# rwth-i6/rasr

Hardware: AMD Instinct MI355X
Metric: acoustic frames scored/sec (1e4-state AM) (higher is better)
Workload: dtype f16+mxfp6 (per f32 product: one f16 MFMA product + one block-scaled fp6 x fp6 MFMA product for both cross terms, f32 accumulate)

## Files before the change

include/amx.h:

```cpp
#ifndef RASR_AMD_AMX_H
#define RASR_AMD_AMX_H

#include <stddef.h>
#include <stdint.h>

#ifdef __cplusplus
extern "C" {
#endif

typedef enum {
    AMX_OK              = 0,
    AMX_ERR_INVALID     = -1,
    AMX_ERR_UNSUPPORTED = -2,
    AMX_ERR_DEVICE      = -3,
    AMX_ERR_STATE       = -4
} amx_status;

typedef struct amx_ctx  amx_ctx;
typedef struct amx_mfcc amx_mfcc;
typedef struct amx_mfcc_plan amx_mfcc_plan;
typedef struct amx_gmm  amx_gmm;
typedef struct amx_ffnn amx_ffnn;


// ... 289 lines not shown
    int                 n_pre;
    const int*          pre_type;
    const float* const* pre_mean;
    const float* const* pre_stddev;
    const int*          maxout_groups;
    const int* const*   maxout_sizes;
} amx_ffnn_layers;
int amx_ffnn_create_ex(amx_ctx* ctx, const amx_ffnn_model* model, const amx_ffnn_layers* ext, amx_ffnn** out);
void amx_ffnn_destroy(amx_ffnn* h);
int  amx_ffnn_input_dim(const amx_ffnn* h);
int  amx_ffnn_output_dim(const amx_ffnn* h);
int amx_ffnn_score(amx_ffnn* h, const float* feats_host, int T, float* scores_host);
int amx_ffnn_score_dev(amx_ffnn* h, const float* feats_dev, int feats_stride, int T, float* scores_dev);
int amx_ffnn_wait_dev(amx_ffnn* h);
int amx_ffnn_precision(const amx_ffnn* h, double* mx_block_ratio);
enum { AMX_NN_TOP_LINEAR = 0, AMX_NN_TOP_SOFTMAX = 1 };
int amx_ffnn_forward_dev(amx_ffnn* h, const float* feats_dev, int feats_stride, int T, float* out_dev, int top);
int amx_ffnn_score_stats_dev(amx_ffnn* h, const float* feats_dev, int feats_stride, int T, float* scores_dev,
                             uint32_t* best_state_dev, unsigned long long* state_counts_dev, double* score_sum_dev);

int amx_ffnn_hidden_dim(const amx_ffnn* h);
int amx_ffnn_forward_hidden_dev(amx_ffnn* h, const float* feats_dev, int feats_stride, int T, float* act_dev);
int amx_ffnn_score_on_demand_dev(amx_ffnn* h, const float* act_dev, int n_pairs, const uint32_t* frame_dev, const uint32_t* emission_dev,
                                 float* scores_dev);
int amx_precomputed_score_dev(amx_ctx* ctx, const float* feats_dev, int feats_stride, int T, int n_classes, const int* class_to_output_dev,
                              const float* log_prior_dev, float prior_scale, float* scores_dev);

int amx_class_labels_init(int n_classes, const int* disregard, int n_disregard, int* mapping, int* n_targets);
int amx_nn_vector_read_f32(const char* path, int* n, float** data);
int amx_nn_vector_write_f32(const char* path, int n, const float* data);
// ... 62 lines not shown
```

rasr_amd/_lib.py:

```python
import ctypes as C
import os

_HERE = os.path.dirname(os.path.abspath(__file__))
LIB_PATH = os.environ.get("AMX_LIBRARY", os.path.join(_HERE, "librasr_amd.so"))

AMX_OK, AMX_ERR_INVALID, AMX_ERR_UNSUPPORTED, AMX_ERR_DEVICE, AMX_ERR_STATE = 0, -1, -2, -3, -4
AMX_GMM_MAX, AMX_GMM_SUM, AMX_GMM_BATCH_FLOAT, AMX_GMM_SIMD, AMX_GMM_BATCH_INT, AMX_GMM_PRESELECTION_FLOAT, AMX_GMM_PRESELECTION_INT = 0, 1, 2, 3, 4, 5, 6
AMX_GMM_VITERBI, AMX_GMM_BAUM_WELCH = 0, 1
AMX_ACT_NONE, AMX_ACT_RELU, AMX_ACT_SIGMOID, AMX_ACT_TANH, AMX_ACT_ELU = 0, 1, 2, 3, 4
AMX_NN_PRE_LOGARITHM, AMX_NN_PRE_MEAN_AND_VARIANCE = 1, 2
AMX_NN_MAX_PRE = 4
AMX_PREC_FP32, AMX_PREC_BF16, AMX_PREC_BF16X3, AMX_PREC_F16MX = 0, 1, 2, 3
AMX_NN_TOP_LINEAR, AMX_NN_TOP_SOFTMAX = 0, 1
AMX_ARCHIVE_READ, AMX_ARCHIVE_WRITE = 0, 1
AMX_NORM_MEAN, AMX_NORM_MEAN_AND_VARIANCE = 0, 1


class AmxError(RuntimeError):
    def __init__(self, status, message):
        super().__init__("amx status %d: %s" % (status, message))
        self.status = status


class MfccCfg(C.Structure):
# ... 158 lines not shown
    "amx_pms_read": (C.c_int, [C.c_char_p, C.POINTER(_P)]),
    "amx_pms_write": (C.c_int, [C.POINTER(GmmModel), C.c_char_p]),
    "amx_mixture_set_view": (C.c_int, [_P, C.POINTER(GmmModel)]),
    "amx_mixture_set_destroy": (None, [_P]),
    "amx_ffnn_create": (C.c_int, [_P, C.POINTER(FfnnModel), C.POINTER(_P)]),
    "amx_ffnn_create_ex": (C.c_int, [_P, C.POINTER(FfnnModel), C.POINTER(FfnnLayers), C.POINTER(_P)]),
    "amx_ffnn_destroy": (None, [_P]),
    "amx_ffnn_input_dim": (C.c_int, [_P]),
    "amx_ffnn_output_dim": (C.c_int, [_P]),
    "amx_ffnn_score": (C.c_int, [_P, _P, C.c_int, _P]),
    "amx_ffnn_score_dev": (C.c_int, [_P, _P, C.c_int, C.c_int, _P]),
    "amx_device_clocks_dev": (C.c_int, [_P, _P]),
    "amx_device_clocks_xcd_dev": (C.c_int, [_P, _P]),
    "amx_ffnn_wait_dev": (C.c_int, [_P]),
    "amx_ffnn_precision": (C.c_int, [_P, C.POINTER(C.c_double)]),
    "amx_ffnn_score_stats_dev": (C.c_int, [_P, _P, C.c_int, C.c_int, _P, _P, _P, _P]),
    "amx_ffnn_hidden_dim": (C.c_int, [_P]),
    "amx_dc_detection": (C.c_int, [_P, C.c_longlong, C.c_double, C.c_double, C.c_float, C.c_double, C.c_int, C.c_int, _P, _P, C.c_longlong, _P]),
    "amx_ffnn_forward_hidden_dev": (C.c_int, [_P, _P, C.c_int, C.c_int, _P]),
    "amx_ffnn_forward_dev": (C.c_int, [_P, _P, C.c_int, C.c_int, _P, C.c_int]),
    "amx_ffnn_score_on_demand_dev": (C.c_int, [_P, _P, C.c_int, _P, _P, _P]),
    "amx_precomputed_score_dev": (C.c_int, [_P, _P, C.c_int, C.c_int, C.c_int, _P, _P, C.c_float, _P]),
    "amx_class_labels_init": (C.c_int, [C.c_int, _P, C.c_int, _P, C.POINTER(C.c_int)]),
    "amx_nn_vector_read_f32": (C.c_int, [C.c_char_p, C.POINTER(C.c_int), C.POINTER(_P)]),
    "amx_nn_vector_write_f32": (C.c_int, [C.c_char_p, C.c_int, _P]),
    "amx_nn_vector_read_s32": (C.c_int, [C.c_char_p, C.POINTER(C.c_int), C.POINTER(_P)]),
    "amx_nn_vector_write_s32": (C.c_int, [C.c_char_p, C.c_int, _P]),
    "amx_nn_vector_read_u32": (C.c_int, [C.c_char_p, C.POINTER(C.c_int), C.POINTER(_P)]),
    "amx_nn_matrix_read": (C.c_int, [C.c_char_p, C.POINTER(C.c_int), C.POINTER(C.c_int), C.POINTER(_P)]),
    "amx_nn_matrix_write": (C.c_int, [C.c_char_p, C.c_int, C.c_int, _P]),
# ... 59 lines not shown
```

rasr_amd/csrc/ffnn.hip:

```cpp
#include "common.hpp"

#include <hip/hip_bf16.h>

#include <algorithm>
#include <map>
#include <tuple>
#include <type_traits>
#include <cmath>
#include <cstring>

namespace amx {

typedef __attribute__((ext_vector_type(8))) short bf16x8;
typedef __attribute__((ext_vector_type(16))) float f32x16;
typedef unsigned short                              bf16_t;

typedef float  f32x2 __attribute__((ext_vector_type(2)));
typedef float  f32x4 __attribute__((ext_vector_type(4)));
typedef __bf16 bf16x2 __attribute__((ext_vector_type(2)));

__device__ __forceinline__ unsigned pack_bf16(float lo, float hi) {
    f32x2 v = {lo, hi};
    return __builtin_bit_cast(unsigned, __builtin_convertvector(v, bf16x2));
}
// ... 1325 lines not shown
        const void *feats, *scores, *best, *counts, *sum;
        hipStream_t stream;
        int         stride, T, stats;
        bool operator<(const GraphKey& o) const {
            return std::tie(feats, scores, best, counts, sum, stream, stride, T, stats) <
                   std::tie(o.feats, o.scores, o.best, o.counts, o.sum, o.stream, o.stride, o.T, o.stats);
        }
    };
    std::map<GraphKey, hipGraphExec_t> graphs;
    float *d_host_f = nullptr, *d_host_s = nullptr;
    size_t host_f_cap = 0, host_s_cap = 0;
    int    use_graphs = 1;
    int    gemm_persistent = 1;
    int    gemm_cfg       = -1;
    int    chunk          = 32768;
    int    mx_stagger     = 0;
    int    mx_dbg         = 0;
    int    mx_ksplit      = 1;
    float*    d_ks_ws  = nullptr;
    size_t    ks_ws_cap = 0;
    unsigned* h_overflow = nullptr;
    unsigned* d_overflow = nullptr;
    amx::PreOps         pre{};
    std::vector<float*> d_pre;
    std::vector<int>    mo_groups;
    std::vector<int*>   d_mo_off, d_mo_size;
    int    mo_width = 0;
    float* d_mo     = nullptr;
    size_t elt() const { return precision == AMX_PREC_FP32 ? 4 : 2; }
    bool   mfma_bf16() const { return precision != AMX_PREC_FP32; }
// ... 185 lines not shown
        case 11:
            if constexpr (LAST)
                launch_bf16<CfgS3, ACT, LAST>(h, l, x, ldx, out, ldo, T, Tpad);
            else
                launch_bf16<CfgS3L, ACT, LAST>(h, l, x, ldx, out, ldo, T, Tpad);
            break;
        default: launch_bf16<CfgA, ACT, LAST>(h, l, x, ldx, out, ldo, T, Tpad); break;
    }
}

using MfgL = amx::mx::MxCfg<256, 256, 2, 4, 3>;
using MfgLP = amx::mx::MxCfg<256, 256, 2, 4, 3, 4>;
using MfgLH = amx::mx::MxCfg<256, 256, 2, 4, 3, 0, 4>;
using MfgLF = amx::mx::MxCfg<256, 256, 2, 4, 3, 4, 4>;
using MfgLQ = amx::mx::MxCfg<256, 256, 2, 4, 3, 0, 0, 1, 0, 1>;
using MfgLW = amx::mx::MxCfg<256, 256, 2, 2, 3, 0, 0, 1, 0, 2>;
using MfgA = amx::mx::MxCfg<128, 128, 2, 2, 3>;
using MfgS = amx::mx::MxCfg<128, 64, 2, 2, 8, 0, 0, 2>;
using MfgS4 = amx::mx::MxCfg<128, 64, 2, 2, 4>;
using MfgSL = amx::mx::MxCfg<128, 64, 2, 2, 8, 0, 0, 2, 4>;
using MfgS8 = amx::mx::MxCfg<128, 64, 4, 2, 8, 0, 0, 2>;
using Mfg64 = amx::mx::MxCfg<64, 64, 2, 2, 8, 0, 0, 4, 4>;
using MfgSP = amx::mx::MxCfg<128, 64, 2, 2, 8, 0, 0, 2, 4, 3>;

template<class C, int ACT, bool LAST>
void launch_mx(amx_ffnn* h, int l, const void* x, int xkts, void* out, int ldo, int T, int Tpad, int n_valid) {
    const int ntn = h->Npad[l] / C::BN, ntt = Tpad / C::BT;
    const int gt = h->group_t >= 0 ? h->group_t : (C::BN == 256 ? 16 : 8), gn = h->group_n >= 0 ? h->group_n : (C::BN == 256 ? 8 : 2);
    constexpr int lds_bytes = amx::gemm_scratch_bytes<C, LAST>() + C::BN * 4;
    static_assert(lds_bytes <= 160 * 1024, "LDS budget");
// ... 96 lines not shown
            cfg = 8;
        else if (t128 >= ncu)
            cfg = 0;
        else if (t64 > ncu && t64 <= 2 * ncu)
            cfg = 6;
        else if (!LAST && 2 * t64 <= ncu && h->mx_ksplit <= 1)
            cfg = 14;
        else
            cfg = 3;
    }
    switch (cfg) {
        case 2: launch_mx<MfgL, ACT, LAST>(h, l, x, xkts, out, ldo, T, Tpad, n_valid); break;
        case 4: launch_mx<MfgLP, ACT, LAST>(h, l, x, xkts, out, ldo, T, Tpad, n_valid); break;
        case 5: launch_mx<MfgLH, ACT, LAST>(h, l, x, xkts, out, ldo, T, Tpad, n_valid); break;
        case 7: launch_mx<MfgLF, ACT, LAST>(h, l, x, xkts, out, ldo, T, Tpad, n_valid); break;
        case 8: launch_mx<MfgLQ, ACT, LAST>(h, l, x, xkts, out, ldo, T, Tpad, n_valid); break;
        case 9: launch_mx<MfgLW, ACT, LAST>(h, l, x, xkts, out, ldo, T, Tpad, n_valid); break;
        case 3:
            if constexpr (LAST)
                launch_mx<MfgS, ACT, LAST>(h, l, x, xkts, out, ldo, T, Tpad, n_valid);
            else
                launch_mx<MfgSP, ACT, LAST>(h, l, x, xkts, out, ldo, T, Tpad, n_valid);
            break;
        case 6: launch_mx<MfgS4, ACT, LAST>(h, l, x, xkts, out, ldo, T, Tpad, n_valid); break;
        case 12: launch_mx<MfgS8, ACT, LAST>(h, l, x, xkts, out, ldo, T, Tpad, n_valid); break;
        case 14:
            if constexpr (LAST)
                launch_mx<MfgS, ACT, LAST>(h, l, x, xkts, out, ldo, T, Tpad, n_valid);
            else
                launch_mx<Mfg64, ACT, LAST>(h, l, x, xkts, out, ldo, T, Tpad, n_valid);
            break;
// ... 89 lines not shown
        const amx::MaxoutSrc<decltype(a)::value> src{h->d_mo, h->out[l], h->d_mo_off[l], h->d_mo_size[l]};
        if (export_f32) {
            const int blocks = (int)std::min<long long>(4096, ((long long)Trows * Kp + 255) / 256);
            hipLaunchKernelGGL(amx::pack_input_f32<decltype(src)>, dim3(blocks), dim3(256), 0, h->ctx->stream, src, T, G, (float*)dst, Kp, Trows);
        }
        else
            pack_operand(h, src, T, G, dst, Kp, Trows);
    });
    AMX_HIP(hipGetLastError());
    return AMX_OK;
}

}

extern "C" {

int amx_ffnn_create(amx_ctx* ctx, const amx_ffnn_model* m, amx_ffnn** out) {
    return amx_ffnn_create_ex(ctx, m, nullptr, out);
}

int amx_ffnn_create_ex(amx_ctx* ctx, const amx_ffnn_model* m, const amx_ffnn_layers* ext, amx_ffnn** out) {
    AMX_REQUIRE(ctx && m && out, AMX_ERR_INVALID, "amx_ffnn_create: NULL argument");
    *out = nullptr;
    AMX_REQUIRE(m->n_layers >= 1 && m->in_dim && m->out_dim && m->W && m->bias && m->activation, AMX_ERR_INVALID,
                "amx_ffnn_create: empty network");
    AMX_REQUIRE(m->precision == AMX_PREC_FP32 || m->precision == AMX_PREC_BF16 || m->precision == AMX_PREC_BF16X3 ||
                        m->precision == AMX_PREC_F16MX,
                AMX_ERR_INVALID, "amx_ffnn_create: unknown precision");
    const int        n_pre = ext ? ext->n_pre : 0;
    std::vector<int> mo_groups((size_t)m->n_layers, 0);
// ... 84 lines not shown
            if (o < 0)
                continue;
            memcpy(&Wmap[(size_t)e * K], m->W[L0] + (size_t)o * K, (size_t)K * 4);
            bmap[e] = m->bias[L0] ? m->bias[L0][o] : 0.f;
            pmap[e] = m->log_prior ? m->log_prior[o] : 0.f;
        }
        out_dim[L0] = m->n_classes;
        Wl[L0]      = Wmap.data();
        bl[L0]      = bmap.data();
        if (m->log_prior)
            prior = pmap.data();
    }

    amx::Tuning tune;
    {
        static const char* const keys[] = {"tile", "graph", "persistent", "group", "chunk", "stagger", "mx_dbg", "mx_fallback", "ksplit", nullptr};
        if (!tune.parse(m->tuning, keys, "amx_ffnn_create"))
            return AMX_ERR_INVALID;
    }
    int t_tile, t_graph, t_persistent, t_chunk, t_mx_dbg, t_stagger, t_group_t = -1, t_group_n = -1, t_ksplit = 1;
    std::string t_mx_fallback;
    {
        const char* who = "amx_ffnn_create";
        static const char* const fallbacks[] = {"auto", "off", nullptr};
        if (!tune.get_word("mx_fallback", "auto", fallbacks, &t_mx_fallback, who) || !tune.get_int("ksplit", 1, 1, 4, &t_ksplit, who))
            return AMX_ERR_INVALID;
        AMX_REQUIRE(t_ksplit == 1 || t_ksplit == 4, AMX_ERR_INVALID, "amx_ffnn_create: tuning ksplit=%d: expected 1 | 4", t_ksplit);
        AMX_REQUIRE(t_ksplit == 1 || m->precision == AMX_PREC_F16MX, AMX_ERR_UNSUPPORTED, "amx_ffnn_create: tuning ksplit exists for AMX_PREC_F16MX only");
        if (!tune.get_int("tile", -1, -1, 14, &t_tile, who) || !tune.get_int("graph", 0, 0, 1, &t_graph, who) ||
            !tune.get_int("persistent", 1, 0, 1, &t_persistent, who) || !tune.get_int("chunk", 32768, 256, 1 << 24, &t_chunk, who) ||
            !tune.get_int("mx_dbg", 0, 0, 1 << 16, &t_mx_dbg, who) || !tune.get_int("stagger", 0, 0, 100000, &t_stagger, who))
            return AMX_ERR_INVALID;
        if (tune.has("group")) {
            const std::string g = tune.kv["group"];
            char              tail = 0;
            AMX_REQUIRE(sscanf(g.c_str(), "%dx%d%c", &t_group_t, &t_group_n, &tail) == 2 && t_group_t >= 1 && t_group_n >= 1 && t_group_t <= 4096 &&
                                t_group_n <= 4096,
                        AMX_ERR_INVALID, "amx_ffnn_create: tuning group=%s: expected <frame tiles>x<output tiles>, e.g. 16x8", g.c_str());
        }
    }
    int    prec = m->precision;
    double mx_ratio = 0.0;
    if (prec == AMX_PREC_F16MX) {
        for (int l = 0; l < m->n_layers; ++l) {
            const int    K = m->in_dim[l], N = out_dim[l];
            const float* W = Wl[l];
// ... 25 lines not shown
    }
    amx_ffnn* h  = new amx_ffnn;
    h->ctx       = ctx;
    h->n_layers  = m->n_layers;
    h->precision = prec;
    h->requested_precision = m->precision;
    h->mx_block_ratio      = mx_ratio;
    h->class_mapped = class_mapped;
    h->gemm_cfg        = t_tile;
    h->use_graphs      = t_graph;
    h->gemm_persistent = t_persistent;
    h->chunk           = t_chunk;
    h->mx_dbg          = t_mx_dbg;
    h->mx_stagger      = t_stagger;
    h->mx_ksplit       = t_ksplit;
    h->group_t         = t_group_t;
    h->group_n         = t_group_n;
    hipSetDevice(ctx->device);
    const int kmult = prec == AMX_PREC_F16MX ? amx::mx::TK : (prec != AMX_PREC_FP32) ? amx::BK : amx::FK;
    if (prec == AMX_PREC_F16MX) {
        if (hipHostMalloc((void**)&h->h_overflow, 4, hipHostMallocMapped) != hipSuccess ||
            hipHostGetDevicePointer((void**)&h->d_overflow, h->h_overflow, 0) != hipSuccess) {
            (void)hipGetLastError();
            amx::set_error("amx_ffnn_create: cannot allocate the overflow flag");
            amx_ffnn_destroy(h);
            return AMX_ERR_DEVICE;
        }
        *h->h_overflow = 0;
    }
    long      best_flops = -1;
// ... 565 lines not shown
```

rasr_amd/csrc/ffnn_mx.hpp:

```cpp
#pragma once

namespace amx {
namespace mx {

typedef _Float16 f16x8 __attribute__((ext_vector_type(8)));
typedef unsigned u32x4 __attribute__((ext_vector_type(4)));
typedef unsigned u32x2 __attribute__((ext_vector_type(2)));
typedef _Float16 f16x2 __attribute__((ext_vector_type(2)));
typedef _Float16 f16x16 __attribute__((ext_vector_type(16)));
typedef _Float16 f16x32 __attribute__((ext_vector_type(32)));
typedef float    f32v16 __attribute__((ext_vector_type(16)));
typedef unsigned u32x6 __attribute__((ext_vector_type(6)));
typedef int      v8i __attribute__((ext_vector_type(8)));

constexpr int TK    = 32;
constexpr int R_OFF = 16384;
constexpr int BLK   = 24576;

__host__ __device__ constexpr int pos16(int u) {
    return 8 * (2 * (u >> 4) + ((u >> 2) & 1)) + 4 * ((u >> 3) & 1) + (u & 3);
}
__host__ __device__ inline int h_off(int r, int c) {
    return r * 64 + ((c ^ ((r >> 2) & 3)) << 4);
}
__host__ __device__ inline int r_off(int r, int half) {
    return R_OFF + half * 4096 + r * 16;
}

__host__ __device__ inline int block_exponent(float max_abs) {
    unsigned u;
#if defined(__HIP_DEVICE_COMPILE__)
    u = __float_as_uint(max_abs);
#else
    memcpy(&u, &max_abs, 4);
#endif
    const int e = (int)((u >> 23) & 0xffu);
    return e < 14 ? 14 : e;
}

static inline unsigned fp6_code_host(float v, int sbyte) {
    const double a = std::fabs((double)v) * std::ldexp(1.0, 127 - sbyte);
// ... 2 lines not shown
        code = 31;
    else {
        const double step = a >= 4.0 ? 0.5 : a >= 2.0 ? 0.25 : 0.125;
        const double qv   = std::nearbyint(a / step) * step;
        if (qv >= 4.0)
            code = 24 + (unsigned)((qv - 4.0) / 0.5);
        else if (qv >= 2.0)
            code = 16 + (unsigned)((qv - 2.0) / 0.25);
        else
            code = (unsigned)(qv / 0.125);
    }
    return code | (std::signbit(v) ? 32u : 0u);
}

static inline void pack_weights_host(const float* W, int n_rows, int K, int ld, int Rpad, int KT, std::vector<unsigned char>& out) {
    out.assign((size_t)(Rpad / 256) * KT * BLK, 0);
    auto block_max = [&](int n, int kt) {
        float m = 0.f;
        if (n < n_rows)
            for (int u = 0; u < 32; ++u) {
                const int k = kt * 32 + u;
                if (k < K)
                    m = std::fmax(m, std::fabs(W[(size_t)n * ld + k]));
            }
        return m;
    };
    for (int n = 0; n < n_rows; ++n) {
        const int rb = n >> 8, r = n & 255;
        for (int kt = 0; kt < KT; ++kt) {
            unsigned char* blk = out.data() + ((size_t)rb * KT + kt) * BLK;
            float          v[32], lo[32];
            _Float16       hi[32];
            for (int u = 0; u < 32; ++u) {
                const int k = kt * 32 + u;
                v[u]        = k < K ? W[(size_t)n * ld + k] : 0.f;
                hi[u]       = (_Float16)v[u];
                lo[u]       = v[u] - (float)hi[u];
            }
            const int ec = block_exponent(std::fmax(block_max(n, kt), block_max(n ^ 32, kt)));
            unsigned  rec[2][4] = {{0, 0, 0, (unsigned)(ec - 2)}, {0, 0, 0, (unsigned)(ec - 2)}};
            for (int u = 0; u < 32; ++u) {
                const int p = pos16(u), chunk = p >> 3, half = chunk & 1, f = 8 * (chunk >> 1) + (p & 7);
                memcpy(blk + h_off(r, chunk) + (p & 7) * 2, &hi[u], 2);
                const unsigned code = fp6_code_host(lo[u], ec - 13);
                const int      bit = 6 * f, d = bit >> 5, sh = bit & 31;
                rec[half][d] |= code << sh;
                if (sh > 26)
                    rec[half][d + 1] |= code >> (32 - sh);
            }
            memcpy(blk + r_off(r, 0), rec[0], 16);
            memcpy(blk + r_off(r, 1), rec[1], 16);
        }
    }
}

struct LanePack {
    uint4 h0, h1, rec;
};

__device__ __forceinline__ unsigned pk_f16(float a, float b) {
    f16x2 v = {(_Float16)a, (_Float16)b};
    return __builtin_bit_cast(unsigned, v);
}

__device__ __forceinline__ LanePack lane_pack(const float (&a)[16], int ec, int sbyte) {
    LanePack o;
// ... 42 lines not shown
            }
        m = fmaxf(m, __shfl_xor(m, 1, 64));
        if (!(m < 65520.f))
            *overflow = 1u;
        const int ec = block_exponent(m);
        lane_store(out + ((size_t)(t >> 8) * KT + kt) * BLK, t & 255, hh, lane_pack(a, ec, ec - 13));
    }
}

template<int ACT>
__global__ __launch_bounds__(256) void neg_act_kernel(float* __restrict__ x, long long n) {
    for (long long i = (long long)blockIdx.x * 256 + threadIdx.x; i < n; i += (long long)gridDim.x * 256)
        x[i] = activate<ACT>(-x[i]);
}

template<int BN_, int BT_, int WN_, int WT_, int STAGES_, int PF_ = 0, int IW_ = 0, int U_ = 1, int LW_ = 0, int PIPE_ = 0>
struct MxCfg {
    static constexpr int BN = BN_, BT = BT_, WN = WN_, WT = WT_, STAGES = STAGES_;
    static constexpr int PIPE = PIPE_;
    static_assert(PIPE_ == 0 || (PIPE_ == 1 && U_ == 1 && LW_ == 0 && PF_ == 0 && IW_ == 0 && STAGES_ == 3 && WN_ * WT_ == 8) ||
                      (PIPE_ == 2 && U_ == 1 && LW_ == 0 && PF_ == 0 && IW_ == 0 && STAGES_ == 3 && WN_ * WT_ == 4 && BN_ / WN_ == 128 && BT_ / WT_ == 128) ||
                      (PIPE_ == 3 && U_ == 2 && LW_ > 0 && STAGES_ >= 2 * U_ + 1),
                  "ping-pong K loop: eight waves, every one of them issuing, plain three-stage ring; self-pipelined: four waves of 128 x 128; "
                  "read-ahead: loader waves, two K-tiles per barrier, a ring of at least three iterations");
    static constexpr int PF = PF_;
    static constexpr int U = U_;
    static_assert(U_ >= 1 && U_ <= 4 && STAGES_ >= 2 * U_, "ring: U K-tiles being read + at least U in flight");
    static_assert(PF_ == 0 || (BN_ == 256 && BT_ == 256 && WN_ * WT_ == 8), "the prefetch walks whole 256-row blocks with six waves");
    static constexpr int NW = WN * WT, LW = LW_, THREADS = (NW + LW_) * 64, PLANES = 1;
    static_assert(LW_ == 0 || (IW_ == 0 && PF_ == 0), "loader waves replace the issuing-wave variants");
    static constexpr bool SKEW = false, SPREAD = false;
    static constexpr int MI = BN / WN / 32, MJ = BT / WT / 32;
    static constexpr int A_R = BN * 64, A_BYTES = BN * 96;
    static constexpr int B_R = BT * 64, B_BYTES = BT * 96;
    static constexpr int STAGE_BYTES = A_BYTES + B_BYTES, LDS_BYTES = STAGES * STAGE_BYTES;
    static constexpr int A_PIECES = BN / 16 + BN / 32, B_PIECES = BT / 16 + BT / 32;
    static constexpr int TOTAL = A_PIECES + B_PIECES;
    static constexpr int IW  = LW_ > 0 ? LW_ : IW_ > 0 ? IW_ : NW;
    static constexpr int PPW = (TOTAL + IW - 1) / IW;
    static constexpr int NHI = TOTAL % IW;
    static constexpr bool PF_FREE = PF_ > 0 && IW_ > 0;
    static_assert(PF_ == 0 || IW_ == 0 || IW_ * 2 == WN_ * WT_, "free prefetch: half of the waves issue the DMA");
    static_assert(BN % 64 == 0 && BT % 64 == 0 && 256 % BN == 0 && 256 % BT == 0, "tiles are whole record pieces of a 256-row block");
    static_assert(STAGES >= 2 && STAGES <= 8 && (STAGES - 2) * (PPW + (PF_ > 0 ? 1 : 0)) + 1 < 64, "vmcnt immediate");
};

template<class C>
__device__ __forceinline__ void piece_offsets(int p, int ha, int hb, int& src, int& dst, bool& is_b) {
    is_b = p >= C::A_PIECES;
    if (!is_b) {
        if (p < C::BN / 16) {
            src = (ha * (C::BN / 16) + p) * 1024;
            dst = p * 1024;
        }
        else {
            const int j = p - C::BN / 16, half = j / (C::BN / 64), gq = j % (C::BN / 64);
            src = R_OFF + half * 4096 + (ha * (C::BN / 64) + gq) * 1024;
            dst = C::A_R + half * (C::BN * 16) + gq * 1024;
        }
    }
    else {
        const int q = p - C::A_PIECES;
        if (q < C::BT / 16) {
            src = (hb * (C::BT / 16) + q) * 1024;
            dst = C::A_BYTES + q * 1024;
// ... 105 lines not shown
            tile_n = 0;
        }
        auto tile_stamp = [&](int phase) {
#ifdef AMX_LAB
            if constexpr ((DBG & 2048) != 0) {
                const int nth = (vi - (int)blockIdx.x) / (int)gridDim.x;
                if (blockIdx.x == 0 && nth < 4 && tid == 0 && (!LAST || n_tiles_total > 1000)) {
                    mx_tile_stamps[(nth * 3 + phase) * 2]     = __builtin_amdgcn_s_memtime();
                    mx_tile_stamps[(nth * 3 + phase) * 2 + 1] = __builtin_amdgcn_s_memrealtime();
                }
            }
#endif
        };
        tile_stamp(0);
        const int   n0 = tile_n * C::BN, t0 = tile_t * C::BT;
        const char* wblk = W + (size_t)(n0 >> 8) * KT * BLK;
        const char* xblk = X + (size_t)(t0 >> 8) * xkts * BLK;
        const int   ha = (n0 & 255) / C::BN, hb = (t0 & 255) / C::BT;
        const int KT_all = KT;
        if (reduce)
            KT = 0;
        if (KSPLIT && ks > 1) {
            const int per = ((KT_all + ks - 1) / ks + C::U - 1) / C::U * C::U, kt_lo = min(kgroup * per, KT_all);
            KT   = min(per, KT_all - kt_lo);
            wblk += (size_t)kt_lo * BLK;
            xblk += (size_t)kt_lo * BLK;
        }

        int  p_src[C::PPW], p_dst[C::PPW];
        bool p_b[C::PPW];
#pragma unroll
        for (int q = 0; q < C::PPW; ++q) {
            const int p = q * C::IW + iwave;
            if (p < C::TOTAL && issuer)
                piece_offsets<C>(p, ha, hb, p_src[q], p_dst[q], p_b[q]);
            else {
                p_src[q] = p_dst[q] = 0;
                p_b[q]              = false;
            }
        }
        const unsigned voff = (unsigned)lane * 16u;
        const unsigned lds_base = (unsigned)(uintptr_t)lds;
        auto piece = [&](int q, int slot, int kt) {
            if ((q == C::PPW - 1 && !hi_wave) || !issuer)
                return;
            int ktm = kt;
            if constexpr ((DBG & 1024) != 0) {
                ktm = kt + (tile_n * 5 + tile_t * 3) % KT;
                ktm = ktm >= KT ? ktm - KT : ktm;
            }
            const char*    src = (p_b[q] ? xblk : wblk) + (size_t)ktm * BLK + p_src[q];
            const unsigned dst = (unsigned)__builtin_amdgcn_readfirstlane((int)(lds_base + slot * C::STAGE_BYTES + p_dst[q]));
            asm volatile("s_mov_b32 m0, %2\n\ts_nop 0\n\tglobal_load_lds_dwordx4 %0, %1" ::"v"(voff), "s"(src), "s"(dst) : "memory");
        };
        float    pf_reg  = 0.f;
        const bool pf_wave = C::PF > 0 && (C::PF_FREE ? wave >= C::IW : wave < 6);
        auto prefetch = [&](int kt) {
            if constexpr (C::PF > 0) {
                if (pf_wave) {
                    const int ktc = min(kt, KT - 1);
                    if constexpr (C::PF_FREE) {
#pragma unroll
                        for (int c = 0; c < 2; ++c) {
                            const int ch = (wave - C::IW) + 4 * c;
                            if (ch < 6) {
                                const char* p = (ch < 3 ? wblk : xblk) + (size_t)ktc * BLK + (ch % 3) * 8192;
                                asm volatile("global_load_dword %0, %1, %2" : "+v"(pf_reg) : "v"((unsigned)lane * 128u), "s"(p) : "memory");
                            }
                        }
                    }
                    else {
                        const char* p = (wave < 3 ? wblk : xblk) + (size_t)ktc * BLK + (wave % 3) * 8192;
                        asm volatile("global_load_dword %0, %1, %2" : "+v"(pf_reg) : "v"((unsigned)lane * 128u), "s"(p) : "memory");
                    }
                }
            }
        };
        auto stage = [&](int slot, int kt) {
#pragma unroll
            for (int q = 0; q < C::PPW; ++q)
                piece(q, slot, kt);
            prefetch(kt + C::PF);
        };

        f32x16 acc[C::MI][C::MJ];
#pragma unroll
        for (int i = 0; i < C::MI; ++i)
// ... 5 lines not shown
        float* s_bias = (float*)(lds + gemm_scratch_bytes<C, LAST>());
        for (int i = tid; i < C::BN; i += C::THREADS)
            s_bias[i] = bias[n0 + i];

#pragma unroll
        for (int s = 0; s < ((C::PIPE == 1 || C::PIPE == 2) ? C::STAGES : C::STAGES - C::U); ++s)
            if (s < KT)
                stage(s, s);
        const int frow = lane & 31, fk = lane >> 5;
        const int a_row = wn * WNR + frow, b_row = wt * WTT + frow;
        struct Frag {
            f16x8 a[2][C::MI], b[2][C::MJ];
            uint4 ra[C::MI], rb[C::MJ];
        };
        Frag fr[C::U];
        auto reads = [&](int kt, Frag& F) {
            auto& a  = F.a;
            auto& b  = F.b;
            auto& ra = F.ra;
            auto& rb = F.rb;
            const char* ab = lds + (kt % C::STAGES) * C::STAGE_BYTES;
            const char* bb = ab + C::A_BYTES;
#pragma unroll
            for (int ks = 0; ks < 2; ++ks) {
#pragma unroll
                for (int i = 0; i < C::MI; ++i)
                    a[ks][i] = *(const f16x8*)(ab + h_off(a_row + 32 * i, 2 * ks + fk));
#pragma unroll
                for (int j = 0; j < C::MJ; ++j)
                    b[ks][j] = *(const f16x8*)(bb + h_off(b_row + 32 * j, 2 * ks + fk));
            }
#pragma unroll
            for (int i = 0; i < C::MI; ++i)
                ra[i] = __builtin_bit_cast(uint4, *(const f16x8*)(ab + C::A_R + fk * (C::BN * 16) + (a_row + 32 * i) * 16));
#pragma unroll
            for (int j = 0; j < C::MJ; ++j)
                rb[j] = __builtin_bit_cast(uint4, *(const f16x8*)(bb + C::B_R + fk * (C::BT * 16) + (b_row + 32 * j) * 16));
        };
        constexpr int N_MFMA = 3 * C::MI * C::MJ, GAP = N_MFMA / C::PPW > 0 ? N_MFMA / C::PPW : 1;
        int           dma_kt = -1;
        constexpr int N_SIDE = 3 * (C::MI + C::MJ);
        auto side_read = [&](Frag& F, int side_kt, int p) {
            const char* ab = lds + (side_kt % C::STAGES) * C::STAGE_BYTES;
            const char* bb = ab + C::A_BYTES;
            if (p < C::MI)
                F.a[0][p] = *(const f16x8*)(ab + h_off(a_row + 32 * p, fk));
            else if (p < C::MI + C::MJ)
                F.b[0][p - C::MI] = *(const f16x8*)(bb + h_off(b_row + 32 * (p - C::MI), fk));
            else if (p < 2 * C::MI + C::MJ)
// ... 49 lines not shown
            if constexpr ((DBG & 32) != 0) {
#pragma unroll
                for (int i = 0; i < C::MI; ++i)
                    keep_alive(ra[i].x), keep_alive(ra[i].y), keep_alive(ra[i].z), keep_alive(ra[i].w);
#pragma unroll
                for (int j = 0; j < C::MJ; ++j)
                    keep_alive(rb[j].x), keep_alive(rb[j].y), keep_alive(rb[j].z), keep_alive(rb[j].w);
                for (int m = 0; m < C::MI * C::MJ; ++m)
                    after_mfma();
                if (dma_kt >= 0)
                    prefetch(dma_kt + C::PF);
                dma_kt = -1;
                return;
            }
            v8i av[C::MI], bv[C::MJ];
            if constexpr (C::MI % 2 == 0) {
#pragma unroll
                for (int i = 0; i < C::MI; i += 2) {
                    u32x6 q;
                    if constexpr ((DBG & 128) != 0)
                        q = u32x6{ra[i].y, ra[i].z, ra[i].x, ra[i + 1].y, ra[i + 1].z, ra[i + 1].x};
                    else
                        q = q_fields_pair(a[0][i], a[1][i], a[0][i + 1], a[1][i + 1], ra[i].w);
                    av[i]     = v8i{(int)q[0], (int)q[1], (int)q[2], (int)ra[i].x, (int)ra[i].y, (int)ra[i].z, 0, 0};
                    av[i + 1] = v8i{(int)q[3], (int)q[4], (int)q[5], (int)ra[i + 1].x, (int)ra[i + 1].y, (int)ra[i + 1].z, 0, 0};
                }
            }
            else {
#pragma unroll
                for (int i = 0; i < C::MI; ++i) {
                    u32x6 q;
                    if constexpr ((DBG & 128) != 0)
                        q = u32x6{ra[i].y, ra[i].z, ra[i].x, 0, 0, 0};
                    else
                        q = q_fields<true>(a[0][i], a[1][i], ra[i].w);
                    av[i] = v8i{(int)q[0], (int)q[1], (int)q[2], (int)ra[i].x, (int)ra[i].y, (int)ra[i].z, 0, 0};
                }
            }
            if constexpr (C::MJ % 2 == 0 && (DBG & 128) == 0) {
#pragma unroll
                for (int j = 0; j < C::MJ; j += 2) {
                    u32x4 x0[2], x1[2];
#pragma unroll
                    for (int ks = 0; ks < 2; ++ks) {
                        x0[ks] = __builtin_bit_cast(u32x4, b[ks][j]);
                        x1[ks] = __builtin_bit_cast(u32x4, b[ks][j + 1]);
#pragma unroll
                        for (int d = 0; d < 4; ++d) {
                            const u32x2 sw = __builtin_amdgcn_permlane32_swap(x0[ks][d], x1[ks][d], false, false);
                            x0[ks][d]      = sw[0];
                            x1[ks][d]      = sw[1];
// ... 21 lines not shown
                    else
                        q = q_fields<false>(b[0][j], b[1][j], rb[j].w + 11u);
                    bv[j] = v8i{(int)rb[j].x, (int)rb[j].y, (int)rb[j].z, (int)q[3], (int)q[4], (int)q[5], 0, 0};
                }
            }
#pragma unroll
            for (int i = 0; i < C::MI; ++i)
#pragma unroll
                for (int j = 0; j < C::MJ; ++j) {
                    if constexpr ((DBG & 8) != 0)
                    {
                        keep_alive(av[i]);
                        keep_alive(bv[j]);
                    }
                    else
                        acc[i][j] = __builtin_amdgcn_mfma_scale_f32_32x32x64_f8f6f4(av[i], bv[j], acc[i][j], 2, 2, 0, (int)ra[i].w, 0, (int)rb[j].w);
                    after_mfma();
                }
            if (dma_kt >= 0)
                prefetch(dma_kt + C::PF);
            dma_kt = -1;
        };
        auto products = [&](Frag& F) { products_side(F, F, 0, false); };
        auto products_ahead = [&](Frag& F, Frag& SIDE, int side_kt, bool side_on) {
            static_assert(C::PIPE != 3 || (C::MI == 2 && C::MJ == 1), "read-ahead K loop: 64 x 32 wave tiles");
            if constexpr (C::MI == 2 && C::MJ == 1) {
                u32x6 qa, qb;
                if constexpr ((DBG & 128) != 0) {
                    qa = u32x6{F.ra[0].y, F.ra[0].z, F.ra[0].x, F.ra[1].y, F.ra[1].z, F.ra[1].x};
                    qb = u32x6{0, 0, 0, F.rb[0].y, F.rb[0].z, F.rb[0].x};
                }
// ... 65 lines not shown
        };
        auto refill = [&](int kt) {
            if constexpr (C::SPREAD == ((DBG & 512) != 0)) {
                if (dma_kt >= 0)
                    stage(dma_kt % C::STAGES, dma_kt);
                dma_kt = -1;
            }
            stamp(kt, 1);
        };
        if constexpr (C::PIPE == 2) {
            static_assert(DBG == 0 || DBG == 2048, "the self-pipelined K loop has no ablation variants");
            static_assert(C::NHI == 0 && C::IW == C::NW && C::MI == 4 && C::MJ == 4, "every wave issues PPW pieces");
            auto await_tile = [&](int ahead_tiles) { mx_wait_ahead<C::PPW, 0, 2>(ahead_tiles); };
            const unsigned vdma = (unsigned)lane * 16u;
            auto dma = [&](int q, int slot, int kt) {
                const char*    src = (p_b[q] ? xblk : wblk) + (size_t)kt * BLK + p_src[q];
                const unsigned dst = (unsigned)__builtin_amdgcn_readfirstlane((int)(lds_base + slot * C::STAGE_BYTES + p_dst[q]));
                asm volatile("s_mov_b32 m0, %2\n\ts_nop 0\n\tglobal_load_lds_dwordx4 %0, %1" ::"v"(vdma), "s"(src), "s"(dst) : "memory");
            };
            Frag& F = fr[0];
            asm volatile("s_waitcnt lgkmcnt(0)" ::: "memory");
            await_tile(min(2, KT - 1));
            __builtin_amdgcn_s_barrier();
            reads(0, F);
            auto f16_products = [&](int ks, int i) {
#pragma unroll
                for (int j = 0; j < 4; ++j)
                    acc[i][j] = __builtin_amdgcn_mfma_f32_32x32x16_f16(F.a[ks][i], F.b[ks][j], acc[i][j], 0, 0, 0);
            };
            auto frame_swaps = [&](int j, u32x4 (&x0)[2], u32x4 (&x1)[2]) {
#pragma unroll
// ... 375 lines not shown
```

Measured before the change: 5.058 million.

## Store precomputed fp6 quantization of weight f16 parts in packed blocks

After: 4.988 million. 1.4% lower.

```diff
diff --git a/include/amx.h b/include/amx.h
--- a/include/amx.h
+++ b/include/amx.h
@@ -327,6 +327,7 @@
 int amx_ffnn_score_dev(amx_ffnn* h, const float* feats_dev, int feats_stride, int T, float* scores_dev);
 int amx_ffnn_wait_dev(amx_ffnn* h);
 int amx_ffnn_precision(const amx_ffnn* h, double* mx_block_ratio);
+int amx_ffnn_pack_weights_f16mx(const float* W, int n_rows, int K, unsigned char* out, size_t out_bytes, size_t* needed);
 enum { AMX_NN_TOP_LINEAR = 0, AMX_NN_TOP_SOFTMAX = 1 };
 int amx_ffnn_forward_dev(amx_ffnn* h, const float* feats_dev, int feats_stride, int T, float* out_dev, int top);
 int amx_ffnn_score_stats_dev(amx_ffnn* h, const float* feats_dev, int feats_stride, int T, float* scores_dev,
diff --git a/rasr_amd/_lib.py b/rasr_amd/_lib.py
--- a/rasr_amd/_lib.py
+++ b/rasr_amd/_lib.py
@@ -196,6 +196,7 @@
     "amx_device_clocks_xcd_dev": (C.c_int, [_P, _P]),
     "amx_ffnn_wait_dev": (C.c_int, [_P]),
     "amx_ffnn_precision": (C.c_int, [_P, C.POINTER(C.c_double)]),
+    "amx_ffnn_pack_weights_f16mx": (C.c_int, [_P, C.c_int, C.c_int, _P, C.c_size_t, C.POINTER(C.c_size_t)]),
     "amx_ffnn_score_stats_dev": (C.c_int, [_P, _P, C.c_int, C.c_int, _P, _P, _P, _P]),
     "amx_ffnn_hidden_dim": (C.c_int, [_P]),
     "amx_dc_detection": (C.c_int, [_P, C.c_longlong, C.c_double, C.c_double, C.c_float, C.c_double, C.c_int, C.c_int, _P, _P, C.c_longlong, _P]),
diff --git a/rasr_amd/csrc/ffnn.hip b/rasr_amd/csrc/ffnn.hip
--- a/rasr_amd/csrc/ffnn.hip
+++ b/rasr_amd/csrc/ffnn.hip
@@ -1363,6 +1363,7 @@
     int    gemm_persistent = 1;
     int    gemm_cfg       = -1;
     int    chunk          = 32768;
+    int    mx_wq          = 1;
     int    mx_stagger     = 0;
     int    mx_dbg         = 0;
     int    mx_ksplit      = 1;
@@ -1578,6 +1579,7 @@
 using MfgLH = amx::mx::MxCfg<256, 256, 2, 4, 3, 0, 4>;
 using MfgLF = amx::mx::MxCfg<256, 256, 2, 4, 3, 4, 4>;
 using MfgLQ = amx::mx::MxCfg<256, 256, 2, 4, 3, 0, 0, 1, 0, 1>;
+using MfgLQW = amx::mx::MxCfg<256, 256, 2, 4, 3, 0, 0, 1, 0, 1, 1>;
 using MfgLW = amx::mx::MxCfg<256, 256, 2, 2, 3, 0, 0, 1, 0, 2>;
 using MfgA = amx::mx::MxCfg<128, 128, 2, 2, 3>;
 using MfgS = amx::mx::MxCfg<128, 64, 2, 2, 8, 0, 0, 2>;
@@ -1704,7 +1706,12 @@
         case 4: launch_mx<MfgLP, ACT, LAST>(h, l, x, xkts, out, ldo, T, Tpad, n_valid); break;
         case 5: launch_mx<MfgLH, ACT, LAST>(h, l, x, xkts, out, ldo, T, Tpad, n_valid); break;
         case 7: launch_mx<MfgLF, ACT, LAST>(h, l, x, xkts, out, ldo, T, Tpad, n_valid); break;
-        case 8: launch_mx<MfgLQ, ACT, LAST>(h, l, x, xkts, out, ldo, T, Tpad, n_valid); break;
+        case 8:
+            if (h->mx_wq)
+                launch_mx<MfgLQW, ACT, LAST>(h, l, x, xkts, out, ldo, T, Tpad, n_valid);
+            else
+                launch_mx<MfgLQ, ACT, LAST>(h, l, x, xkts, out, ldo, T, Tpad, n_valid);
+            break;
         case 9: launch_mx<MfgLW, ACT, LAST>(h, l, x, xkts, out, ldo, T, Tpad, n_valid); break;
         case 3:
             if constexpr (LAST)
@@ -1824,6 +1831,21 @@
 }
 
 extern "C" {
+
+int amx_ffnn_pack_weights_f16mx(const float* W, int n_rows, int K, unsigned char* out, size_t out_bytes, size_t* needed) {
+    AMX_REQUIRE(W && n_rows > 0 && K > 0, AMX_ERR_INVALID, "amx_ffnn_pack_weights_f16mx: empty matrix");
+    const int    Np = pad_to(n_rows, 256), Kp = pad_to(K, amx::mx::TK);
+    const size_t n  = (size_t)(Np / 256) * (Kp / 32) * amx::mx::WBLK;
+    if (needed)
+        *needed = n;
+    if (!out)
+        return AMX_OK;
+    AMX_REQUIRE(out_bytes >= n, AMX_ERR_INVALID, "amx_ffnn_pack_weights_f16mx: %zu bytes given, %zu needed", out_bytes, n);
+    std::vector<unsigned char> pk;
+    amx::mx::pack_weights_host(W, n_rows, K, K, Np, Kp / 32, pk);
+    memcpy(out, pk.data(), n);
+    return AMX_OK;
+}
 
 int amx_ffnn_create(amx_ctx* ctx, const amx_ffnn_model* m, amx_ffnn** out) {
     return amx_ffnn_create_ex(ctx, m, nullptr, out);
@@ -1938,11 +1960,11 @@
 
     amx::Tuning tune;
     {
-        static const char* const keys[] = {"tile", "graph", "persistent", "group", "chunk", "stagger", "mx_dbg", "mx_fallback", "ksplit", nullptr};
+        static const char* const keys[] = {"tile", "graph", "persistent", "group", "chunk", "stagger", "mx_dbg", "mx_fallback", "ksplit", "wq", nullptr};
         if (!tune.parse(m->tuning, keys, "amx_ffnn_create"))
             return AMX_ERR_INVALID;
     }
-    int t_tile, t_graph, t_persistent, t_chunk, t_mx_dbg, t_stagger, t_group_t = -1, t_group_n = -1, t_ksplit = 1;
+    int t_tile, t_graph, t_persistent, t_chunk, t_mx_dbg, t_stagger, t_group_t = -1, t_group_n = -1, t_ksplit = 1, t_wq = 1;
     std::string t_mx_fallback;
     {
         const char* who = "amx_ffnn_create";
@@ -1953,7 +1975,8 @@
         AMX_REQUIRE(t_ksplit == 1 || m->precision == AMX_PREC_F16MX, AMX_ERR_UNSUPPORTED, "amx_ffnn_create: tuning ksplit exists for AMX_PREC_F16MX only");
         if (!tune.get_int("tile", -1, -1, 14, &t_tile, who) || !tune.get_int("graph", 0, 0, 1, &t_graph, who) ||
             !tune.get_int("persistent", 1, 0, 1, &t_persistent, who) || !tune.get_int("chunk", 32768, 256, 1 << 24, &t_chunk, who) ||
-            !tune.get_int("mx_dbg", 0, 0, 1 << 16, &t_mx_dbg, who) || !tune.get_int("stagger", 0, 0, 100000, &t_stagger, who))
+            !tune.get_int("mx_dbg", 0, 0, 1 << 16, &t_mx_dbg, who) || !tune.get_int("stagger", 0, 0, 100000, &t_stagger, who) ||
+            !tune.get_int("wq", 1, 0, 1, &t_wq, who))
             return AMX_ERR_INVALID;
         if (tune.has("group")) {
             const std::string g = tune.kv["group"];
@@ -2009,6 +2032,7 @@
     h->mx_dbg          = t_mx_dbg;
     h->mx_stagger      = t_stagger;
     h->mx_ksplit       = t_ksplit;
+    h->mx_wq           = t_wq;
     h->group_t         = t_group_t;
     h->group_n         = t_group_n;
     hipSetDevice(ctx->device);
diff --git a/rasr_amd/csrc/ffnn_mx.hpp b/rasr_amd/csrc/ffnn_mx.hpp
--- a/rasr_amd/csrc/ffnn_mx.hpp
+++ b/rasr_amd/csrc/ffnn_mx.hpp
@@ -16,6 +16,9 @@
 constexpr int TK    = 32;
 constexpr int R_OFF = 16384;
 constexpr int BLK   = 24576;
+constexpr int QR_OFF = BLK;
+constexpr int WS_OFF = QR_OFF + 2 * 256 * 24;
+constexpr int WBLK   = WS_OFF + 256;
 
 __host__ __device__ constexpr int pos16(int u) {
     return 8 * (2 * (u >> 4) + ((u >> 2) & 1)) + 4 * ((u >> 3) & 1) + (u & 3);
@@ -25,6 +28,12 @@
 }
 __host__ __device__ inline int r_off(int r, int half) {
     return R_OFF + half * 4096 + r * 16;
+}
+__host__ __device__ inline int qr_off(int r, int half) {
+    return QR_OFF + half * (256 * 24) + r * 24;
+}
+__host__ __device__ inline int ws_off(int r) {
+    return WS_OFF + ((r >> 7) * 32 + (r & 31)) * 4 + ((r >> 6) & 1);
 }
 
 __host__ __device__ inline int block_exponent(float max_abs) {
@@ -57,7 +66,7 @@
 }
 
 static inline void pack_weights_host(const float* W, int n_rows, int K, int ld, int Rpad, int KT, std::vector<unsigned char>& out) {
-    out.assign((size_t)(Rpad / 256) * KT * BLK, 0);
+    out.assign((size_t)(Rpad / 256) * KT * WBLK, 0);
     auto block_max = [&](int n, int kt) {
         float m = 0.f;
         if (n < n_rows)
@@ -71,7 +80,7 @@
     for (int n = 0; n < n_rows; ++n) {
         const int rb = n >> 8, r = n & 255;
         for (int kt = 0; kt < KT; ++kt) {
-            unsigned char* blk = out.data() + ((size_t)rb * KT + kt) * BLK;
+            unsigned char* blk = out.data() + ((size_t)rb * KT + kt) * WBLK;
             float          v[32], lo[32];
             _Float16       hi[32];
             for (int u = 0; u < 32; ++u) {
@@ -82,17 +91,26 @@
             }
             const int ec = block_exponent(std::fmax(block_max(n, kt), block_max(n ^ 32, kt)));
             unsigned  rec[2][4] = {{0, 0, 0, (unsigned)(ec - 2)}, {0, 0, 0, (unsigned)(ec - 2)}};
+            unsigned  qrec[2][4] = {{0, 0, 0, 0}, {0, 0, 0, 0}};
             for (int u = 0; u < 32; ++u) {
                 const int p = pos16(u), chunk = p >> 3, half = chunk & 1, f = 8 * (chunk >> 1) + (p & 7);
                 memcpy(blk + h_off(r, chunk) + (p & 7) * 2, &hi[u], 2);
-                const unsigned code = fp6_code_host(lo[u], ec - 13);
+                const unsigned code = fp6_code_host(lo[u], ec - 13), qcode = fp6_code_host((float)hi[u], ec - 2);
                 const int      bit = 6 * f, d = bit >> 5, sh = bit & 31;
                 rec[half][d] |= code << sh;
-                if (sh > 26)
+                qrec[half][d] |= qcode << sh;
+                if (sh > 26) {
                     rec[half][d + 1] |= code >> (32 - sh);
+                    qrec[half][d + 1] |= qcode >> (32 - sh);
+                }
             }
             memcpy(blk + r_off(r, 0), rec[0], 16);
             memcpy(blk + r_off(r, 1), rec[1], 16);
+            for (int half = 0; half < 2; ++half) {
+                memcpy(blk + qr_off(r, half), qrec[half], 12);
+                memcpy(blk + qr_off(r, half) + 12, rec[half], 12);
+            }
+            blk[ws_off(r)] = (unsigned char)(ec - 2);
         }
     }
 }
@@ -165,7 +183,7 @@
         x[i] = activate<ACT>(-x[i]);
 }
 
-template<int BN_, int BT_, int WN_, int WT_, int STAGES_, int PF_ = 0, int IW_ = 0, int U_ = 1, int LW_ = 0, int PIPE_ = 0>
+template<int BN_, int BT_, int WN_, int WT_, int STAGES_, int PF_ = 0, int IW_ = 0, int U_ = 1, int LW_ = 0, int PIPE_ = 0, int WQ_ = 0>
 struct MxCfg {
     static constexpr int BN = BN_, BT = BT_, WN = WN_, WT = WT_, STAGES = STAGES_;
     static constexpr int PIPE = PIPE_;
@@ -182,10 +200,13 @@
     static_assert(LW_ == 0 || (IW_ == 0 && PF_ == 0), "loader waves replace the issuing-wave variants");
     static constexpr bool SKEW = false, SPREAD = false;
     static constexpr int MI = BN / WN / 32, MJ = BT / WT / 32;
-    static constexpr int A_R = BN * 64, A_BYTES = BN * 96;
+    static constexpr int WQ = WQ_;
+    static_assert(WQ_ == 0 || (PIPE_ == 1 && BN_ == 256 && WN_ == 2), "stored q: the ping-pong tile, whole weight blocks, wave tiles of 128 rows");
+    static constexpr int A_R = BN * 64, A_BYTES = WQ ? BN * 64 + 2 * BN * 24 + 256 : BN * 96;
     static constexpr int B_R = BT * 64, B_BYTES = BT * 96;
     static constexpr int STAGE_BYTES = A_BYTES + B_BYTES, LDS_BYTES = STAGES * STAGE_BYTES;
-    static constexpr int A_PIECES = BN / 16 + BN / 32, B_PIECES = BT / 16 + BT / 32;
+    static_assert(LDS_BYTES + BN * 4 <= 163840, "the ring and the tile's bias fit a CU's 160 KB of LDS");
+    static constexpr int A_PIECES = WQ ? BN / 16 + 2 * BN * 24 / 1024 + 1 : BN / 16 + BN / 32, B_PIECES = BT / 16 + BT / 32;
     static constexpr int TOTAL = A_PIECES + B_PIECES;
     static constexpr int IW  = LW_ > 0 ? LW_ : IW_ > 0 ? IW_ : NW;
     static constexpr int PPW = (TOTAL + IW - 1) / IW;
@@ -199,7 +220,11 @@
 template<class C>
 __device__ __forceinline__ void piece_offsets(int p, int ha, int hb, int& src, int& dst, bool& is_b) {
     is_b = p >= C::A_PIECES;
-    if (!is_b) {
+    if (C::WQ && !is_b) {
+        src = p < C::BN / 16 ? p * 1024 : p < C::A_PIECES - 1 ? QR_OFF + (p - C::BN / 16) * 1024 : WS_OFF;
+        dst = p < C::A_PIECES - 1 ? p * 1024 : C::A_BYTES - 256;
+    }
+    else if (!is_b) {
         if (p < C::BN / 16) {
             src = (ha * (C::BN / 16) + p) * 1024;
             dst = p * 1024;
@@ -335,7 +360,7 @@
         };
         tile_stamp(0);
         const int   n0 = tile_n * C::BN, t0 = tile_t * C::BT;
-        const char* wblk = W + (size_t)(n0 >> 8) * KT * BLK;
+        const char* wblk = W + (size_t)(n0 >> 8) * KT * WBLK;
         const char* xblk = X + (size_t)(t0 >> 8) * xkts * BLK;
         const int   ha = (n0 & 255) / C::BN, hb = (t0 & 255) / C::BT;
         const int KT_all = KT;
@@ -344,7 +369,7 @@
         if (KSPLIT && ks > 1) {
             const int per = ((KT_all + ks - 1) / ks + C::U - 1) / C::U * C::U, kt_lo = min(kgroup * per, KT_all);
             KT   = min(per, KT_all - kt_lo);
-            wblk += (size_t)kt_lo * BLK;
+            wblk += (size_t)kt_lo * WBLK;
             xblk += (size_t)kt_lo * BLK;
         }
 
@@ -362,6 +387,7 @@
         }
         const unsigned voff = (unsigned)lane * 16u;
         const unsigned lds_base = (unsigned)(uintptr_t)lds;
+        auto piece_is_b = [&](int q) { return q * C::IW >= C::A_PIECES ? true : (q + 1) * C::IW <= C::A_PIECES ? false : p_b[q]; };
         auto piece = [&](int q, int slot, int kt) {
             if ((q == C::PPW - 1 && !hi_wave) || !issuer)
                 return;
@@ -370,8 +396,14 @@
                 ktm = kt + (tile_n * 5 + tile_t * 3) % KT;
                 ktm = ktm >= KT ? ktm - KT : ktm;
             }
-            const char*    src = (p_b[q] ? xblk : wblk) + (size_t)ktm * BLK + p_src[q];
+            const char*    src = (piece_is_b(q) ? xblk + (size_t)ktm * BLK : wblk + (size_t)ktm * WBLK) + p_src[q];
             const unsigned dst = (unsigned)__builtin_amdgcn_readfirstlane((int)(lds_base + slot * C::STAGE_BYTES + p_dst[q]));
+            if constexpr (C::WQ != 0) {
+                if (q == (C::A_PIECES - 1) / C::IW && iwave == (C::A_PIECES - 1) % C::IW) {
+                    asm volatile("s_mov_b32 m0, %2\n\ts_nop 0\n\tglobal_load_lds_dword %0, %1" ::"v"((unsigned)lane * 4u), "s"(src), "s"(dst) : "memory");
+                    return;
+                }
+            }
             asm volatile("s_mov_b32 m0, %2\n\ts_nop 0\n\tglobal_load_lds_dwordx4 %0, %1" ::"v"(voff), "s"(src), "s"(dst) : "memory");
         };
         float    pf_reg  = 0.f;
@@ -385,13 +417,13 @@
                         for (int c = 0; c < 2; ++c) {
                             const int ch = (wave - C::IW) + 4 * c;
                             if (ch < 6) {
-                                const char* p = (ch < 3 ? wblk : xblk) + (size_t)ktc * BLK + (ch % 3) * 8192;
+                                const char* p = (ch < 3 ? wblk + (size_t)ktc * WBLK : xblk + (size_t)ktc * BLK) + (ch % 3) * 8192;
                                 asm volatile("global_load_dword %0, %1, %2" : "+v"(pf_reg) : "v"((unsigned)lane * 128u), "s"(p) : "memory");
                             }
                         }
                     }
                     else {
-                        const char* p = (wave < 3 ? wblk : xblk) + (size_t)ktc * BLK + (wave % 3) * 8192;
+                        const char* p = (wave < 3 ? wblk + (size_t)ktc * WBLK : xblk + (size_t)ktc * BLK) + (wave % 3) * 8192;
                         asm volatile("global_load_dword %0, %1, %2" : "+v"(pf_reg) : "v"((unsigned)lane * 128u), "s"(p) : "memory");
                     }
                 }
@@ -427,6 +459,8 @@
             uint4 ra[C::MI], rb[C::MJ];
         };
         Frag fr[C::U];
+        u32x2    wq_qr[C::MI][3];
+        unsigned wq_ws = 0;
         auto reads = [&](int kt, Frag& F) {
             auto& a  = F.a;
             auto& b  = F.b;
@@ -443,9 +477,19 @@
                 for (int j = 0; j < C::MJ; ++j)
                     b[ks][j] = *(const f16x8*)(bb + h_off(b_row + 32 * j, 2 * ks + fk));
             }
-#pragma unroll
-            for (int i = 0; i < C::MI; ++i)
-                ra[i] = __builtin_bit_cast(uint4, *(const f16x8*)(ab + C::A_R + fk * (C::BN * 16) + (a_row + 32 * i) * 16));
+            if constexpr (C::WQ != 0) {
+#pragma unroll
+                for (int i = 0; i < C::MI; ++i)
+#pragma unroll
+                    for (int d = 0; d < 3; ++d)
+                        wq_qr[i][d] = *(const u32x2*)(ab + C::A_R + fk * (C::BN * 24) + (a_row + 32 * i) * 24 + 8 * d);
+                wq_ws = *(const unsigned*)(ab + C::A_BYTES - 256 + (wn * 32 + frow) * 4);
+            }
+            else {
+#pragma unroll
+                for (int i = 0; i < C::MI; ++i)
+                    ra[i] = __builtin_bit_cast(uint4, *(const f16x8*)(ab + C::A_R + fk * (C::BN * 16) + (a_row + 32 * i) * 16));
+            }
 #pragma unroll
             for (int j = 0; j < C::MJ; ++j)
                 rb[j] = __builtin_bit_cast(uint4, *(const f16x8*)(bb + C::B_R + fk * (C::BT * 16) + (b_row + 32 * j) * 16));
@@ -525,7 +569,15 @@
                 return;
             }
             v8i av[C::MI], bv[C::MJ];
-            if constexpr (C::MI % 2 == 0) {
+            int sa[C::MI];
+            if constexpr (C::WQ != 0) {
+#pragma unroll
+                for (int i = 0; i < C::MI; ++i) {
+                    av[i] = v8i{(int)wq_qr[i][0][0], (int)wq_qr[i][0][1], (int)wq_qr[i][1][0], (int)wq_qr[i][1][1], (int)wq_qr[i][2][0], (int)wq_qr[i][2][1], 0, 0};
+                    sa[i] = (int)(i < 2 ? wq_ws : wq_ws >> 8);
+                }
+            }
+            else if constexpr (C::MI % 2 == 0) {
 #pragma unroll
                 for (int i = 0; i < C::MI; i += 2) {
                     u32x6 q;
@@ -535,6 +587,8 @@
                         q = q_fields_pair(a[0][i], a[1][i], a[0][i + 1], a[1][i + 1], ra[i].w);
                     av[i]     = v8i{(int)q[0], (int)q[1], (int)q[2], (int)ra[i].x, (int)ra[i].y, (int)ra[i].z, 0, 0};
                     av[i + 1] = v8i{(int)q[3], (int)q[4], (int)q[5], (int)ra[i + 1].x, (int)ra[i + 1].y, (int)ra[i + 1].z, 0, 0};
+                    sa[i]     = (int)ra[i].w;
+                    sa[i + 1] = (int)ra[i + 1].w;
                 }
             }
             else {
@@ -546,6 +600,7 @@
                     else
                         q = q_fields<true>(a[0][i], a[1][i], ra[i].w);
                     av[i] = v8i{(int)q[0], (int)q[1], (int)q[2], (int)ra[i].x, (int)ra[i].y, (int)ra[i].z, 0, 0};
+                    sa[i] = (int)ra[i].w;
                 }
             }
             if constexpr (C::MJ % 2 == 0 && (DBG & 128) == 0) {
@@ -597,7 +652,7 @@
                         keep_alive(bv[j]);
                     }
                     else
-                        acc[i][j] = __builtin_amdgcn_mfma_scale_f32_32x32x64_f8f6f4(av[i], bv[j], acc[i][j], 2, 2, 0, (int)ra[i].w, 0, (int)rb[j].w);
+                        acc[i][j] = __builtin_amdgcn_mfma_scale_f32_32x32x64_f8f6f4(av[i], bv[j], acc[i][j], 2, 2, 0, sa[i], 0, (int)rb[j].w);
                     after_mfma();
                 }
             if (dma_kt >= 0)
@@ -693,7 +748,7 @@
             auto await_tile = [&](int ahead_tiles) { mx_wait_ahead<C::PPW, 0, 2>(ahead_tiles); };
             const unsigned vdma = (unsigned)lane * 16u;
             auto dma = [&](int q, int slot, int kt) {
-                const char*    src = (p_b[q] ? xblk : wblk) + (size_t)kt * BLK + p_src[q];
+                const char*    src = (piece_is_b(q) ? xblk + (size_t)kt * BLK : wblk + (size_t)kt * WBLK) + p_src[q];
                 const unsigned dst = (unsigned)__builtin_amdgcn_readfirstlane((int)(lds_base + slot * C::STAGE_BYTES + p_dst[q]));
                 asm volatile("s_mov_b32 m0, %2\n\ts_nop 0\n\tglobal_load_lds_dwordx4 %0, %1" ::"v"(vdma), "s"(src), "s"(dst) : "memory");
             };
```
